# INDA25PlusPlus/rsoderh-raytracing

Hardware: AMD Instinct MI355X
Metric: Mrays/s, house.toml 1920x1080 256spp 8-bounce (higher is better)
Workload: dtype f32; 1 GPU; house.toml 1920x1080 256 spp 8 bounces, synthetic 2048x1024 HDRI env; parallelism=single GPU

## Files before the change

rsoderh-raytracing_amd/csrc/hip/rt_wavepool.h:

```cpp
#pragma once
#include "rt_device.h"
#include "rt_coop.h"
#include "rt_cold_layout.h"

enum HotField { H_OX, H_OY, H_OZ, H_EX, H_EY, H_EZ, H_SX, H_SY, H_SZ, H_T, H_CT, H_COUNT };
enum CtBits : uint32_t {
    F_SHADOW = 8u,
    F_EXT = 16u,
    F_NEE = 32u,
    F_OCCLUDED = 64u,
    CT_FLAGS = 120u,
    CT_SHIFT = 7u
};
#define RT_FLAT_BOUNCE_SHIFT 8u
#define RT_FLAT_BOUNCE_BITS 0xffff00u
#define RT_FLAT_RESUMED (1u << 24)
#define RT_FLAT_MAX_BOUNCES 0xffffu
static_assert(kColdWideStack == RT_WSTACK && kColdWideStateWords == RT_WSTATE_WORDS && kColdCoopOverflow == RT_COOP_GCAP,
              "rt_cold_layout.h sizes the walks' columns by the walks' own constants");
enum PoolTag { TAG_FREE = 0, TAG_TRACE = 1, TAG_MISS = 2, TAG_SHADE = 3, TAG_FINISH = 4, TAG_IDLE = 6 };
enum PoolStage { ST_GEN = 0, ST_TRACE = 1, ST_MISS = 2, ST_SHADE = 3, ST_FINISH = 4, ST_COUNT = 5 };

__host__ __device__ constexpr uint32_t pool_hot_columns(int trav) { return trav == 6 ? 12u : (uint32_t)H_COUNT; }
__host__ __device__ constexpr uint32_t pool_list_dwords(int trav) { return trav == 6 ? RT_COOP_LCAP : 64u; }
__host__ __device__ constexpr uint32_t pool_wave_lds_dwords(int trav, uint32_t pool) { return pool_hot_columns(trav) * pool + pool_list_dwords(trav) + (trav == 6 ? RT_COOP_NCAP + RT_COOP_MAP : 0u); }
template <uint32_t POOL, int TRAV>
struct PoolLayout {
    static constexpr uint32_t kSlotsPerLane = (POOL + 63u) / 64u;
    static constexpr uint32_t kHotDwords = pool_hot_columns(TRAV) * POOL;
    static constexpr uint32_t kListDwords = pool_list_dwords(TRAV);
    static constexpr uint32_t kWaveLdsDwords = pool_wave_lds_dwords(TRAV, POOL);
    static constexpr uint32_t kColdColumns = pool_cold_columns(TRAV);
    static constexpr uint32_t kWaveColdDwords = pool_wave_cold_dwords(TRAV, POOL);
    static constexpr uint32_t kCtColumn = pool_hot_columns(TRAV) - 1u;
};

RT_DEV uint32_t stage_of_tag(uint32_t tag) { return tag; }

#define RT_WAVE_HANDOVER()                                        \
    do {                                                          \
        __builtin_amdgcn_fence(__ATOMIC_RELEASE, "wavefront");    \
        __builtin_amdgcn_wave_barrier();                          \
        __builtin_amdgcn_fence(__ATOMIC_ACQUIRE, "wavefront");    \
    } while (0)

typedef float rt_f3v __attribute__((ext_vector_type(3)));
typedef rt_f3v rt_f3v_a4 __attribute__((aligned(4)));
RT_DEV void store_sample(float *dst, V3 L) { __builtin_nontemporal_store(rt_f3v{L.x, L.y, L.z}, reinterpret_cast<rt_f3v_a4 *>(dst)); }

#ifndef RT_POOL_WAVES_PER_SIMD
#define RT_POOL_WAVES_PER_SIMD 4
#endif
template <int SV> struct PoolView;
template <> struct PoolView<0> { typedef SceneView<false> type; static __device__ __forceinline__ type make(const DevScene &sc) { return make_view<false>(sc); } };
template <> struct PoolView<1> { typedef SceneView<true> type; static __device__ __forceinline__ type make(const DevScene &sc) { return make_view<true>(sc); } };
template <> struct PoolView<2> { typedef SceneViewHybrid type; static __device__ __forceinline__ type make(const DevScene &sc) { return make_view_hybrid(sc); } };

template <int SV, uint32_t BLOCK, uint32_t POOL, int TRAV>
__global__ __launch_bounds__(BLOCK, RT_POOL_WAVES_PER_SIMD) void rt_render_pool_kernel(RenderParams P)
{
    typedef PoolLayout<POOL, TRAV> L;
    constexpr bool kCoop = TRAV == 6;
    constexpr bool kBounceInCt = TRAV == 2;
    constexpr bool kFreshInCt = kBounceInCt;
    constexpr bool kOutHot = kFreshInCt;
    constexpr bool kRngHot = TRAV == 2;
    constexpr uint32_t kTCell = kRngHot ? (uint32_t)H_SX : (uint32_t)H_T;
    constexpr bool kFlatVote = kRngHot && kBounceInCt;
    constexpr bool kPackedMiss = TRAV == 2 || TRAV == 6;
    constexpr bool kGenTrace = TRAV >= 2 && !kCoop;
    const DevScene &sc = P.scene;
    if (SV != 0) stage_scene_lds(sc);
    const typename PoolView<SV>::type S = PoolView<SV>::make(sc);
    const uint32_t lane0 = threadIdx.x & (RT_WAVE - 1);
    constexpr bool kScalarWave = SV == 2 || TRAV == 6;
    const uint32_t wave = kScalarWave ? (uint32_t)__builtin_amdgcn_readfirstlane((int)(threadIdx.x / RT_WAVE)) : threadIdx.x / RT_WAVE;
    uint32_t *const lds32 = reinterpret_cast<uint32_t *>(rt_smem + sc.lds_float4s);
    uint32_t *const W = lds32 + wave * L::kWaveLdsDwords;
    uint32_t *const WCT = W + L::kCtColumn * POOL;
    uint32_t *const list = W + L::kHotDwords;
    uint32_t *const G = P.cold_state + (size_t)(blockIdx.x * (BLOCK / RT_WAVE) + wave) * L::kWaveColdDwords;
    const bool prune = (P.flags & RSRT_FLAG_PRUNE) != 0;
    const bool anyhit_shadow = !(P.flags & RSRT_FLAG_REFERENCE_TRAVERSAL);
    const uint32_t tile_px = P.tile_w * P.tile_h;

#define HOT(f, slot) W[(f) * POOL + (slot)]
#define HOTF(f, slot) as_f(HOT(f, slot))
#define SETHU(f, slot, val) W[(f) * POOL + (slot)] = (val)
#define SETH(f, slot, val) SETHU(f, slot, as_u(val))
#define CT_OF(slot) WCT[(slot)]
#define TAG_OF(slot) (WCT[(slot)] & 7u)
#define SET_TAG(slot, tag) WCT[(slot)] = (uint32_t)(tag)
#define SET_CT(slot, payload, flags, tag) WCT[(slot)] = ((payload) << CT_SHIFT) | (flags) | (uint32_t)(tag)
#define BEST_REF(slot) W[9u * POOL + 2u * (slot)]
#define BEST_T(slot) W[9u * POOL + 2u * (slot) + 1u]
#define COLD(f, slot) G[cold_index(TRAV, POOL, (f), (slot))]
#define COLDF(f, slot) as_f(COLD(f, slot))
#define SETC(f, slot, val) COLD(f, slot) = as_u(val)

    for (uint32_t k = 0; k < L::kSlotsPerLane; k++)
        if (lane0 + 64u * k < POOL) SET_TAG(lane0 + 64u * k, TAG_FREE);
    RT_WAVE_HANDOVER();

    uint32_t chunk_next = 0, chunk_left = 0, chunk_tile_slot0 = 0, chunk_tx0 = 0, chunk_ty0 = 0, chunk_s0 = 0, chunk_p0 = 0;
    bool exhausted = false;
    unsigned long long n_paths = 0, n_ext = 0, n_shadow = 0;
    uint32_t n_work = 0;
#ifdef RT_INSTRUMENT
    DbgCounters dbg;
    for (int i = 0; i < RT_DBG_N; i++) dbg.c[i] = 0;
#endif

#ifdef RT_INSTRUMENT
    unsigned long long t_prev = __builtin_amdgcn_s_memtime();
#define DBG_STAMP(i) do { unsigned long long t_now = __builtin_amdgcn_s_memtime(); if (lane0 == 0) dbg.c[i] += t_now - t_prev; t_prev = t_now; } while (0)
#else
#define DBG_STAMP(i) do { } while (0)
#endif
#if defined(RT_INSTRUMENT) && defined(RT_SHADE_PROFILE)
#define SHADE_STAMP(i) DBG_STAMP(i)
#else
#define SHADE_STAMP(i) do { } while (0)
#endif
    auto ray_end = [&](const uint32_t slot, const uint32_t ct, const Hit &h, const uint32_t cur, const float t_in, const unsigned long long flat_rem) __attribute__((always_inline)) {
        const bool shadow = (ct & F_SHADOW) != 0u;
        const uint32_t bounce_bits = kBounceInCt ? ((ct >> CT_SHIFT) & RT_FLAT_BOUNCE_BITS) : 0u;
        const bool found = TRAV >= 3 ? (h.ref != RT_REF_UNKNOWN) : (h.t < t_in);
        const bool done = cur == RT_END || (kFlatVote && shadow && h.t < RT_INFINITY);
        if (!done && kFlatVote) {
            COLD(C_REM_LO, slot) = (uint32_t)flat_rem;
            COLD(C_REM_HI, slot) = (uint32_t)(flat_rem >> 32);
            if (!shadow) SETH(kTCell, slot, h.t);
            SET_CT(slot, RT_FLAT_RESUMED | bounce_bits | (shadow ? 0u : h.ref), ct & CT_FLAGS, TAG_TRACE);
        } else if (!done) {
            if (!kRngHot) SETH(H_T, slot, h.t);
            if (TRAV != 2 && !shadow && found) COLD(C_REF, slot) = h.ref;
            SET_CT(slot, cur, ct & CT_FLAGS, TAG_TRACE);
        } else if (shadow) {
            n_shadow++;
            if (!kRngHot) SETH(H_T, slot, RT_INFINITY);
            const uint32_t fl = (ct & (F_EXT | F_NEE)) | (h.t < RT_INFINITY ? (uint32_t)F_OCCLUDED : 0u);
            SET_CT(slot, bounce_bits, fl, (ct & F_EXT) ? TAG_TRACE : TAG_FINISH);
        } else {
            n_ext++;
            SETH(kTCell, slot, h.t);
            if (TRAV != 2 && found) COLD(C_REF, slot) = h.ref;
            SET_CT(slot, (TRAV == 2 ? h.ref : 0u) | bounce_bits, ct & (F_NEE | F_OCCLUDED), h.did_hit() ? TAG_SHADE : TAG_MISS);
        }
    };
    auto trace_slot = [&](const uint32_t slot, const uint32_t ct, const V3 o, const V3 d, const bool coherent) __attribute__((always_inline)) {
        const bool shadow = (ct & F_SHADOW) != 0u;
        Hit h;
        uint32_t cur = kBounceInCt ? (kFlatVote ? (ct >> (CT_SHIFT + 24u)) : 0u) : (ct >> CT_SHIFT);
        h.src = SRC_BVH;
        h.t = kRngHot ? RT_INFINITY : HOTF(H_T, slot); h.u = h.v = 0.0f;
        unsigned long long flat_rem = 0ull;
        if (kFlatVote && cur != 0u) {
            flat_rem = ((unsigned long long)COLD(C_REM_HI, slot) << 32) | COLD(C_REM_LO, slot);
            if (!shadow) h.t = HOTF(kTCell, slot);
        }
        h.ref = (TRAV >= 3 && !shadow) ? RT_REF_UNKNOWN : ((kFlatVote && cur != 0u) ? ((ct >> CT_SHIFT) & 63u) : 0u);
        const float t_in = h.t;
        trace_dispatch<TRAV>(DBG_ARG S, sc, o, d, prune, shadow && anyhit_shadow, P.trace_budget, TRAV == 2 ? (kFlatVote ? P.flat_quorum : 0u) : P.descend_quorum,
                             cur, h, TRAV == 2 ? nullptr : &COLD(C_REF, slot), n_work, flat_rem, TRAV >= 4 ? &G[C_WIDE_STATE * POOL + slot] : nullptr, POOL, P.stop_quorum, coherent);
        ray_end(slot, ct, h, cur, t_in, flat_rem);
    };
    for (;;) {
        uint32_t lane = lane0;
        if (kCoop) asm volatile("" : "+v"(lane));
        RT_MARK(0);
        DBG_STAMP(21);
        uint32_t tags[L::kSlotsPerLane];
        uint32_t count[ST_COUNT] = {};
        for (uint32_t k = 0; k < L::kSlotsPerLane; k++) {
            tags[k] = (lane + 64u * k < POOL) ? TAG_OF(lane + 64u * k) : (uint32_t)TAG_IDLE;
            const uint32_t st = stage_of_tag(tags[k]);
            for (uint32_t s = 0; s < ST_COUNT; s++) count[s] += (uint32_t)__popcll(__ballot(st == s));
        }
        if (exhausted) count[ST_GEN] = 0;
        uint32_t best = ST_COUNT, best_n = 0;
        for (uint32_t s = 0; s < ST_COUNT; s++)
            if (count[s] >= best_n && count[s] > 0) { best = s; best_n = count[s]; }
        if (best == ST_COUNT) break;
        uint32_t base = 0;
        for (uint32_t k = 0; k < L::kSlotsPerLane; k++) {
            const bool mine = stage_of_tag(tags[k]) == best;
            const unsigned long long m = __ballot(mine);
            const uint32_t pos = base + (uint32_t)__popcll(m & ((1ull << lane) - 1ull));
            if (mine && pos < L::kListDwords) list[pos] = lane + 64u * k;
            base += (uint32_t)__popcll(m);
        }
        RT_WAVE_HANDOVER();
        const uint32_t n_run = min(best_n, 64u);
        const bool on = lane < n_run;
        const uint32_t slot = on ? list[lane] : 0u;
        const uint32_t dbg_stage = best;
        (void)dbg_stage;
        if (lane == 0) { DBG_ADD(dbg_stage, 1); DBG_ADD(5 + dbg_stage, (kCoop && best == ST_TRACE) ? best_n : n_run); }
        DBG_STAMP(22);
        RT_MARK(1);

        if (best == ST_GEN) {
            RT_MARK(2);
            uint32_t given = 0;
            bool started = false;
            V3 cam_o = v3(0.0f, 0.0f, 0.0f), cam_d = v3(0.0f, 0.0f, 0.0f);
            while (given < n_run && !exhausted) {
                if (chunk_left == 0u) {
                    uint32_t c = 0;
                    if (lane == 0) c = atomicAdd(P.work_counter, 1u);
                    c = __builtin_amdgcn_readfirstlane((int)c);
                    if (c >= P.n_chunks) { exhausted = true; break; }
                    const uint32_t q = c % P.n_subtiles, cb = c / P.n_subtiles;
                    const uint32_t j = cb / P.n_sblocks, b = cb % P.n_sblocks;
                    uint32_t ttx, tty;
                    if (!owned_tile(j, P.rank, P.world, P.skew, P.tiles_x, P.tiles_per_row, ttx, tty)) continue;
                    chunk_tx0 = ttx * P.tile_w;
                    chunk_ty0 = tty * P.tile_h;
                    chunk_tile_slot0 = j * tile_px;
                    chunk_s0 = b * P.samples_per_chunk;
                    chunk_p0 = q * P.chunk_px;
                    chunk_next = 0;
                    chunk_left = min(P.samples_per_chunk, P.sample_count - chunk_s0) * P.chunk_px;
                }
                const uint32_t take = min(n_run - given, chunk_left);
                if (on && lane >= given && lane < given + take) {
                    const uint32_t item = chunk_next + (lane - given);
                    const uint32_t ks = item / P.chunk_px, p = chunk_p0 + item % P.chunk_px;
                    const uint32_t px = chunk_tx0 + p % P.tile_w, py = chunk_ty0 + p / P.tile_w;
                    if (px < P.width && py < P.height) {
                        const uint32_t srel = chunk_s0 + ks;
                        PathState ps;
                        start_path(P, px, py, P.sample_begin + srel, ps);
                        SETH(H_OX, slot, ps.o.x); SETH(H_OY, slot, ps.o.y); SETH(H_OZ, slot, ps.o.z);
                        SETH(H_EX, slot, ps.d.x); SETH(H_EY, slot, ps.d.y); SETH(H_EZ, slot, ps.d.z);
                        if (kRngHot) SETHU(H_T, slot, ps.rng);
                        else if (!kCoop) SETH(H_T, slot, RT_INFINITY);
                        if (!kFreshInCt) {
                            SETC(C_TX, slot, 1.0f); SETC(C_TY, slot, 1.0f); SETC(C_TZ, slot, 1.0f);
                            SETC(C_LX, slot, 0.0f); SETC(C_LY, slot, 0.0f); SETC(C_LZ, slot, 0.0f);
                            SETC(C_LASTPDF, slot, 1.0f);
                        }
                        if (!kRngHot) COLD(C_RNG, slot) = ps.rng;
                        if (!kBounceInCt) COLD(C_BOUNCE, slot) = 0u;
                        if (kOutHot) SETHU(H_SY, slot, srel * P.n_slots + chunk_tile_slot0 + p);
                        else COLD(C_OUT, slot) = srel * P.n_slots + chunk_tile_slot0 + p;
                        if (kGenTrace) { started = true; cam_o = ps.o; cam_d = ps.d; }
                        else SET_CT(slot, 0u, F_EXT, TAG_TRACE);
                        n_paths++;
                    }
                }
                given += take;
                chunk_next += take;
                chunk_left -= take;
            }
            RT_MARK(3);
            if (kGenTrace && started) trace_slot(slot, (uint32_t)F_EXT | (uint32_t)TAG_TRACE, cam_o, cam_d, true);
            RT_MARK(14);
            if (exhausted) {
                for (uint32_t k = 0; k < L::kSlotsPerLane; k++)
                    if (lane + 64u * k < POOL && TAG_OF(lane + 64u * k) == TAG_FREE) SET_TAG(lane + 64u * k, TAG_IDLE);
            }
        } else if (kCoop && best == ST_TRACE) {
            if constexpr (kCoop) {
                CoopStacks cs;
                cs.ns = list + L::kListDwords; cs.ls = list; cs.gs = G + L::kColdColumns * POOL;
                cs.map = reinterpret_cast<uint16_t *>(cs.ns + RT_COOP_NCAP);
                cs.ns_h = cs.ns_n = cs.ls_n = cs.gs_n = 0u;
                cs.lds_cap = P.coop_lds_cap; cs.lifo_at = P.coop_lifo_at; cs.narrow_at = P.coop_narrow_at; cs.gcap = P.coop_gcap;
                CoopNoCount coop_cc;
                for (uint32_t i0 = 0; i0 < best_n; i0 += 64u) {
                    const bool valid = i0 + lane < best_n;
                    const uint32_t s = list[valid ? i0 + lane : 0u];
                    coop_push_rays<POOL>(W, cs, coop_cc, valid, s, CT_OF(s), (uint32_t)F_EXT, (uint32_t)F_SHADOW);
                }
                coop_trace<POOL>(DBG_ARG S, W, cs, coop_cc, anyhit_shadow, lane, n_work);
                RT_WAVE_HANDOVER();
                uint32_t my_slot[L::kSlotsPerLane];
                bool mine[L::kSlotsPerLane];
                for (uint32_t k = 0; k < L::kSlotsPerLane; k++) { my_slot[k] = lane + 64u * k; mine[k] = tags[k] == (uint32_t)TAG_TRACE; }
                if (cs.overflowed()) {
                    if (lane == 0u) atomicAdd(&P.stats[RT_COOP_STATS + 6u], 1ull);
                    for (uint32_t k = 0; k < L::kSlotsPerLane; k++)
                        if (mine[k]) coop_abandon<POOL>(W, my_slot[k], (uint32_t)F_EXT, (uint32_t)F_SHADOW);
                }
                coop_slow_rays<POOL, L::kSlotsPerLane>(DBG_ARG S, sc, W, mine, my_slot, anyhit_shadow, n_work);
                for (uint32_t k = 0; k < L::kSlotsPerLane; k++) {
                    if (!mine[k]) continue;
                    const uint32_t s = my_slot[k], ct = CT_OF(s);
                    const uint32_t fl = ct & (uint32_t)(F_NEE | F_OCCLUDED);
                    if (ct & F_SHADOW) n_shadow++;
                    if (ct & F_EXT) {
                        n_ext++;
                        SET_CT(s, 0u, fl, as_f(BEST_T(s)) < RT_INFINITY ? TAG_SHADE : TAG_MISS);
                    } else {
                        SET_CT(s, 0u, fl, TAG_FINISH);
                    }
                }
            }
        } else if (best == ST_TRACE) {
            RT_MARK(12);
            if (on) {
                const uint32_t ct = CT_OF(slot);
                const uint32_t dcol = (ct & F_SHADOW) ? (uint32_t)H_SX : (uint32_t)H_EX;
                const V3 o = v3(HOTF(H_OX, slot), HOTF(H_OY, slot), HOTF(H_OZ, slot));
                const V3 d = v3(HOTF(dcol, slot), HOTF(dcol + 1u, slot), HOTF(dcol + 2u, slot));
                trace_slot(slot, ct, o, d, false);
            }
        } else if (best == ST_MISS) {
            RT_MARK2(0);
            if (on) {
                const uint32_t ct = CT_OF(slot);
                const V3 o = v3(HOTF(H_OX, slot), HOTF(H_OY, slot), HOTF(H_OZ, slot));
                const V3 d = v3(HOTF(H_EX, slot), HOTF(H_EY, slot), HOTF(H_EZ, slot));
                float env_u, env_v;
                direction_to_equirectangular_uv(d, env_u, env_v);
                const EnvBilinearFetch sky_fetch = kPackedMiss ? sample_env_bilinear_begin_pmf(P.env, env_u, env_v) : sample_env_bilinear_begin(P.env, env_u, env_v);
                float sky_pmf = 0.0f;
                if (!kPackedMiss) sky_pmf = environment_direction_pmf(P.env, env_u, env_v);
                float last_pdf;
                V3 T, Lr, nee_prev;
                uint32_t out_slot;
                if constexpr (!kFreshInCt) {
                    last_pdf = COLDF(C_LASTPDF, slot);
                    T = v3(COLDF(C_TX, slot), COLDF(C_TY, slot), COLDF(C_TZ, slot));
                    Lr = v3(COLDF(C_LX, slot), COLDF(C_LY, slot), COLDF(C_LZ, slot));
                    nee_prev = v3(COLDF(C_NEEX, slot), COLDF(C_NEEY, slot), COLDF(C_NEEZ, slot));
                    out_slot = COLD(C_OUT, slot);
                } else {
                    const bool fresh = ((ct >> CT_SHIFT) & RT_FLAT_BOUNCE_BITS) == 0u;
                    const uint32_t out_hot = HOT(H_SY, slot);
                    last_pdf = COLDF(C_LASTPDF, slot);
                    T = v3(COLDF(C_TX, slot), COLDF(C_TY, slot), COLDF(C_TZ, slot));
                    Lr = v3(COLDF(C_LX, slot), COLDF(C_LY, slot), COLDF(C_LZ, slot));
                    nee_prev = v3(COLDF(C_NEEX, slot), COLDF(C_NEEY, slot), COLDF(C_NEEZ, slot));
                    out_slot = COLD(C_OUT, slot);
                    if (fresh) {
                        last_pdf = 1.0f;
                        T = v3(1.0f, 1.0f, 1.0f);
                        Lr = v3(0.0f, 0.0f, 0.0f);
                        out_slot = out_hot;
                    }
                }
                Hit h;
                h.t = RT_INFINITY; h.ref = 0; h.src = SRC_BVH; h.u = h.v = 0.0f;
                for (uint32_t i = 0; i < sc.n_spheres; i++) {
                    RT_MARK2(1);
                    float u, v;
                    float t = test_record(S, i, SRC_FB_SPHERE, o, d, u, v);
                    if (t >= 0.0f && t < h.t) { h.t = t; h.ref = i; h.src = SRC_FB_SPHERE; }
                }
                for (uint32_t i = 0; i < sc.n_planes; i++) {
                    RT_MARK2(2);
                    float u, v;
                    float t = test_record(S, i, SRC_FB_PLANE, o, d, u, v);
                    if (t >= 0.0f && t < h.t) { h.t = t; h.ref = i; h.src = SRC_FB_PLANE; }
                }
                RT_MARK2(3);
                if (h.did_hit()) {
                    if (kCoop) BEST_T(slot) = as_u(h.t); else SETH(kTCell, slot, h.t);
                    if (kCoop) {
                        BEST_REF(slot) = h.ref | (h.src << 30);
                        SET_CT(slot, 0u, ct & (F_NEE | F_OCCLUDED), TAG_SHADE);
                    } else if (TRAV == 2) {
                        SET_CT(slot, h.ref | (h.src << 6) | (kBounceInCt ? ((ct >> CT_SHIFT) & RT_FLAT_BOUNCE_BITS) : 0u), ct & (F_NEE | F_OCCLUDED), TAG_SHADE);
                    } else {
                        COLD(C_REF, slot) = h.ref | (h.src << 30);
                        SET_CT(slot, 0u, ct & (F_NEE | F_OCCLUDED), TAG_SHADE);
                    }
                } else {
                    const V3 sky = sample_env_bilinear_finish(sky_fetch);
                    if (kPackedMiss) sky_pmf = env_bilinear_pmf(P.env, sky_fetch, env_u, env_v);
                    const float pdf = sky_pmf / environment_pixel_solid_angle(env_v, P.env);
                    const float w = power_heuristic(last_pdf, pdf);
                    if ((ct & (F_NEE | F_OCCLUDED)) == F_NEE) Lr = Lr + nee_prev;
                    Lr = Lr + T * sky * w;
                    store_sample(P.sample_buf + (size_t)out_slot * 3u, Lr);
                    SET_TAG(slot, TAG_FREE);
                }
            }
        } else if (best == ST_SHADE) {
            RT_MARK2(4);
            if (on) {
                const uint32_t ct = CT_OF(slot);
                const V3 o = v3(HOTF(H_OX, slot), HOTF(H_OY, slot), HOTF(H_OZ, slot));
                const V3 d = v3(HOTF(H_EX, slot), HOTF(H_EY, slot), HOTF(H_EZ, slot));
                Hit h;
                h.t = kCoop ? as_f(BEST_T(slot)) : HOTF(kTCell, slot);
                if (TRAV == 2) {
                    const uint32_t hr = (ct >> CT_SHIFT) & 0xffu;
                    h.ref = hr & 63u; h.src = hr >> 6;
                } else {
                    const uint32_t hr = kCoop ? BEST_REF(slot) : COLD(C_REF, slot);
                    h.ref = hr & 0x3fffffffu; h.src = hr >> 30;
                }
                DBG_ADD(27, (as_u(hit_record(S, h, 0).w) & 3u) == PRIM_TRIANGLE ? 1 : 0); DBG_ADD(31, (as_u(hit_record(S, h, 0).w) & 3u) == PRIM_SPHERE ? 1 : 0);
                uint32_t rng, bounce;
                uint32_t out_slot = 0u;
                V3 T, Lr;
                Surface surf;
                BsdfMaterial mat;
                EnvironmentSample es;
                if constexpr (kRngHot) {
                    rng = HOT(H_T, slot);
                    const EnvironmentPick pick = sample_environment_begin(P.env, rng);
                    T = v3(COLDF(C_TX, slot), COLDF(C_TY, slot), COLDF(C_TZ, slot));
                    Lr = v3(COLDF(C_LX, slot), COLDF(C_LY, slot), COLDF(C_LZ, slot));
                    const V3 nee_prev = v3(COLDF(C_NEEX, slot), COLDF(C_NEEY, slot), COLDF(C_NEEZ, slot));
                    if (kOutHot) out_slot = COLD(C_OUT, slot);
                    bounce = (kBounceInCt ? (ct >> (CT_SHIFT + RT_FLAT_BOUNCE_SHIFT)) : COLD(C_BOUNCE, slot)) + 1u;
                    if (kFreshInCt && bounce == 1u) {
                        T = v3(1.0f, 1.0f, 1.0f);
                        Lr = v3(0.0f, 0.0f, 0.0f);
                        if (kOutHot) out_slot = HOT(H_SY, slot);
                    }
                    SHADE_STAMP(10);
                    hit_barycentrics(S, h, o, d);
                    surf = resolve_hit(S, h, o, d);
                    mat = load_material(S, surf.material_id);
                    SHADE_STAMP(11);
                    es = sample_environment_finish<true>(P.env, rng, pick);
                    SHADE_STAMP(12);
                    if ((ct & (F_NEE | F_OCCLUDED)) == F_NEE) Lr = Lr + nee_prev;
                    Lr = Lr + T * mat.emission;
                } else {
                    hit_barycentrics(S, h, o, d);
                    rng = COLD(C_RNG, slot);
                    T = v3(COLDF(C_TX, slot), COLDF(C_TY, slot), COLDF(C_TZ, slot));
                    Lr = v3(COLDF(C_LX, slot), COLDF(C_LY, slot), COLDF(C_LZ, slot));
                    bounce = (kBounceInCt ? (ct >> (CT_SHIFT + RT_FLAT_BOUNCE_SHIFT)) : COLD(C_BOUNCE, slot)) + 1u;
                    if ((ct & (F_NEE | F_OCCLUDED)) == F_NEE) Lr = Lr + v3(COLDF(C_NEEX, slot), COLDF(C_NEEY, slot), COLDF(C_NEEZ, slot));
                    surf = resolve_hit(S, h, o, d);
                    mat = load_material(S, surf.material_id);
                    Lr = Lr + T * mat.emission;
                    es = sample_environment(P.env, rng);
                }
                const float cos_nee = fmax_(0.0f, dot(surf.normal, es.direction));
                const bool want_shadow = cos_nee > 0.0f && es.pdf > 0.0f;
                const Frame frame = make_frame(surf.normal);
                const V3 wo = to_frame_local(frame, -d);
                V3 nee = v3(0.0f, 0.0f, 0.0f);
                const float g1_o = kRngHot ? g1_ggx(wo.z, mat.alpha) : 0.0f;
                if (want_shadow) {
                    RT_MARK2(5);
                    DBG_WAVE_TICK(23); DBG_ADD(24, 1);
                    const V3 wi = to_frame_local(frame, es.direction);
                    V3 scattering;
                    float pdf_bsdf;
                    if (kRngHot) bsdf_eval_pdf_local<true>(wo, wi, mat, g1_o, scattering, pdf_bsdf);
                    else bsdf_eval_pdf_local(wo, wi, mat, scattering, pdf_bsdf);
                    const float w = power_heuristic(es.pdf, pdf_bsdf);
                    nee = T * w * es.radiance * scattering * cos_nee / es.pdf;
                }
                RT_MARK2(6);
                SHADE_STAMP(13);
                const BsdfSample bs = kRngHot ? bsdf_sample_in_frame<true>(d, surf.normal, frame, wo, mat, g1_o, rng) : bsdf_sample_in_frame(d, surf.normal, frame, wo, mat, rng);
                RT_MARK2(15);
                SHADE_STAMP(14);
                bool finished = false, nee_counts = want_shadow;
                if (bs.dir.x == 0.0f && bs.dir.y == 0.0f && bs.dir.z == 0.0f) {
                    Lr = bs.scattering;
                    nee_counts = false;
                    finished = true;
                } else if (bs.pdf <= 0.0f) {
                    finished = true;
                } else {
                    const float c = fmax_(0.0f, dot(surf.normal, bs.dir));
                    T = T * (bs.scattering * (c / bs.pdf));
                    if (length(T) < 0.001f) finished = true;
                }
                if (bounce >= P.max_bounces) finished = true;
                if (finished && !want_shadow) {
                    store_sample(P.sample_buf + (size_t)(kOutHot ? out_slot : COLD(C_OUT, slot)) * 3u, Lr);
                    SET_TAG(slot, TAG_FREE);
                } else {
                    SETC(C_LX, slot, Lr.x); SETC(C_LY, slot, Lr.y); SETC(C_LZ, slot, Lr.z);
                    if (kOutHot) COLD(C_OUT, slot) = out_slot;
                    if (nee_counts) { SETC(C_NEEX, slot, nee.x); SETC(C_NEEY, slot, nee.y); SETC(C_NEEZ, slot, nee.z); }
                    if (!finished) {
                        SETC(C_LASTPDF, slot, bs.pdf);
                        SETC(C_TX, slot, T.x); SETC(C_TY, slot, T.y); SETC(C_TZ, slot, T.z);
                        if (kRngHot) SETHU(H_T, slot, rng); else COLD(C_RNG, slot) = rng;
                        if (!kBounceInCt) COLD(C_BOUNCE, slot) = bounce;
                        SETH(H_EX, slot, bs.dir.x); SETH(H_EY, slot, bs.dir.y); SETH(H_EZ, slot, bs.dir.z);
                    }
                    if (want_shadow) { SETH(H_SX, slot, es.direction.x); SETH(H_SY, slot, es.direction.y); SETH(H_SZ, slot, es.direction.z); }
                    SETH(H_OX, slot, surf.point.x); SETH(H_OY, slot, surf.point.y); SETH(H_OZ, slot, surf.point.z);
                    if (!kRngHot && !kCoop) SETH(H_T, slot, RT_INFINITY);
                    SET_CT(slot, kBounceInCt ? (bounce << RT_FLAT_BOUNCE_SHIFT) : 0u,
                           (want_shadow ? (uint32_t)F_SHADOW : 0u) | (finished ? 0u : (uint32_t)F_EXT) | (nee_counts ? (uint32_t)F_NEE : 0u), TAG_TRACE);
                }
            }
        } else {
            RT_MARK2(7);
            if (on) {
                const uint32_t ct = CT_OF(slot);
                V3 Lr = v3(COLDF(C_LX, slot), COLDF(C_LY, slot), COLDF(C_LZ, slot));
                if ((ct & (F_NEE | F_OCCLUDED)) == F_NEE) Lr = Lr + v3(COLDF(C_NEEX, slot), COLDF(C_NEEY, slot), COLDF(C_NEEZ, slot));
                store_sample(P.sample_buf + (size_t)COLD(C_OUT, slot) * 3u, Lr);
                SET_TAG(slot, TAG_FREE);
            }
        }
        RT_MARK(15);
        RT_WAVE_HANDOVER();
        DBG_STAMP(16 + dbg_stage);
    }
#undef HOT
#undef HOTF
#undef SETHU
#undef SETH
#undef CT_OF
#undef TAG_OF
#undef SET_TAG
#undef SET_CT
#undef COLD
#undef BEST_REF
#undef BEST_T
#undef COLDF
#undef SETC

    RT_MARK(11);
    unsigned long long n_work64 = n_work;
    for (int off = 32; off > 0; off >>= 1) {
        n_paths += __shfl_down(n_paths, off);
        n_ext += __shfl_down(n_ext, off);
        n_shadow += __shfl_down(n_shadow, off);
        if (TRAV != 2) n_work64 += __shfl_down(n_work64, off);
    }
    if (lane0 == 0) {
        atomicAdd(&P.stats[0], n_paths);
        atomicAdd(&P.stats[1], n_ext);
        atomicAdd(&P.stats[2], n_shadow);
        if (TRAV != 2) atomicAdd(&P.stats[3], n_work64);
    }
#ifdef RT_INSTRUMENT
    for (int i = 0; i < RT_DBG_N; i++) {
        unsigned long long v = dbg.c[i];
        for (int off = 32; off > 0; off >>= 1) v += __shfl_down(v, off);
        if (lane0 == 0 && v) atomicAdd(&P.stats[4 + i], v);
    }
#endif
}
```

Measured before the change: 23240 Mrays/s.

## Track per-stage slot counts incrementally and pick stage via packed max key

For the TRAV==2 wavefront pool, the scheduler now keeps running per-stage counts and updates them after each stage from ballots over only the slots that just ran, instead of re-ballotting every pool slot against every stage each iteration. Stage selection becomes a packed (count<<3|stage) max chain kept in scalar registers, and list compaction uses mbcnt instead of a masked popcount. This is meant to cut scheduler overhead per iteration, at the cost of bookkeeping that must stay exactly in step with tag transitions. Only the default TRAV==2 path uses it, if that is the active traversal.

```diff
diff --git a/rsoderh-raytracing_amd/csrc/hip/rt_pool_pick.h b/rsoderh-raytracing_amd/csrc/hip/rt_pool_pick.h
--- /dev/null
+++ b/rsoderh-raytracing_amd/csrc/hip/rt_pool_pick.h
@@ -0,0 +1,39 @@
+#pragma once
+#include <cstdint>
+
+#if defined(__HIPCC__) || defined(__CUDACC__)
+#define RT_PICK_FN __host__ __device__ inline
+#else
+#define RT_PICK_FN inline
+#endif
+#if defined(__HIP_DEVICE_COMPILE__)
+#define RT_PICK_SCALAR(x) asm volatile("" : "+s"(x))
+#else
+#define RT_PICK_SCALAR(x) (void)(x)
+#endif
+
+constexpr uint32_t kPoolPickStages = 5u;
+
+struct PoolPick {
+    uint32_t best;
+    uint32_t best_n;
+};
+
+RT_PICK_FN uint32_t pool_pick_max(uint32_t a, uint32_t b) { return a > b ? a : b; }
+
+RT_PICK_FN PoolPick pool_pick(uint32_t n_gen, uint32_t n_trace, uint32_t n_miss, uint32_t n_shade, uint32_t n_finish, bool exhausted)
+{
+    uint32_t key = exhausted ? 0u : (n_gen << 3);
+    key = pool_pick_max(key, (n_trace << 3) | 1u);
+    RT_PICK_SCALAR(key);
+    key = pool_pick_max(key, (n_miss << 3) | 2u);
+    RT_PICK_SCALAR(key);
+    key = pool_pick_max(key, (n_shade << 3) | 3u);
+    RT_PICK_SCALAR(key);
+    key = pool_pick_max(key, (n_finish << 3) | 4u);
+    RT_PICK_SCALAR(key);
+    PoolPick p;
+    p.best = key < 8u ? kPoolPickStages : (key & 7u);
+    p.best_n = key >> 3;
+    return p;
+}
diff --git a/rsoderh-raytracing_amd/csrc/hip/rt_wavepool.h b/rsoderh-raytracing_amd/csrc/hip/rt_wavepool.h
--- a/rsoderh-raytracing_amd/csrc/hip/rt_wavepool.h
+++ b/rsoderh-raytracing_amd/csrc/hip/rt_wavepool.h
@@ -2,6 +2,7 @@
 #include "rt_device.h"
 #include "rt_coop.h"
 #include "rt_cold_layout.h"
+#include "rt_pool_pick.h"
 
 enum HotField { H_OX, H_OY, H_OZ, H_EX, H_EY, H_EZ, H_SX, H_SY, H_SZ, H_T, H_CT, H_COUNT };
 enum CtBits : uint32_t {
@@ -20,6 +21,7 @@
               "rt_cold_layout.h sizes the walks' columns by the walks' own constants");
 enum PoolTag { TAG_FREE = 0, TAG_TRACE = 1, TAG_MISS = 2, TAG_SHADE = 3, TAG_FINISH = 4, TAG_IDLE = 6 };
 enum PoolStage { ST_GEN = 0, ST_TRACE = 1, ST_MISS = 2, ST_SHADE = 3, ST_FINISH = 4, ST_COUNT = 5 };
+static_assert(ST_COUNT == kPoolPickStages, "rt_pool_pick.h picks among these stages, in this order");
 
 __host__ __device__ constexpr uint32_t pool_hot_columns(int trav) { return trav == 6 ? 12u : (uint32_t)H_COUNT; }
 __host__ __device__ constexpr uint32_t pool_list_dwords(int trav) { return trav == 6 ? RT_COOP_LCAP : 64u; }
@@ -69,6 +71,9 @@
     constexpr bool kFlatVote = kRngHot && kBounceInCt;
     constexpr bool kPackedMiss = TRAV == 2 || TRAV == 6;
     constexpr bool kGenTrace = TRAV >= 2 && !kCoop;
+    constexpr bool kKeptCounts = TRAV == 2;
+    constexpr bool kKeyPick = TRAV == 2;
+    constexpr bool kMbcnt = TRAV == 2;
     const DevScene &sc = P.scene;
     if (SV != 0) stage_scene_lds(sc);
     const typename PoolView<SV>::type S = PoolView<SV>::make(sc);
@@ -104,6 +109,8 @@
 
     uint32_t chunk_next = 0, chunk_left = 0, chunk_tile_slot0 = 0, chunk_tx0 = 0, chunk_ty0 = 0, chunk_s0 = 0, chunk_p0 = 0;
     bool exhausted = false;
+    uint32_t kept[ST_COUNT] = {POOL, 0u, 0u, 0u, 0u};
+    (void)kept;
     unsigned long long n_paths = 0, n_ext = 0, n_shadow = 0;
     uint32_t n_work = 0;
 #ifdef RT_INSTRUMENT
@@ -172,22 +179,42 @@
         DBG_STAMP(21);
         uint32_t tags[L::kSlotsPerLane];
         uint32_t count[ST_COUNT] = {};
-        for (uint32_t k = 0; k < L::kSlotsPerLane; k++) {
-            tags[k] = (lane + 64u * k < POOL) ? TAG_OF(lane + 64u * k) : (uint32_t)TAG_IDLE;
-            const uint32_t st = stage_of_tag(tags[k]);
-            for (uint32_t s = 0; s < ST_COUNT; s++) count[s] += (uint32_t)__popcll(__ballot(st == s));
+        if constexpr (kKeptCounts) {
+            for (uint32_t k = 0; k < L::kSlotsPerLane; k++)
+                tags[k] = (lane + 64u * k < POOL) ? TAG_OF(lane + 64u * k) : (uint32_t)TAG_IDLE;
+            for (uint32_t s = 0; s < ST_COUNT; s++) count[s] = kept[s];
+#ifdef RT_INSTRUMENT
+            for (uint32_t s = 0; s < ST_COUNT; s++) {
+                uint32_t n = 0;
+                for (uint32_t k = 0; k < L::kSlotsPerLane; k++) n += (uint32_t)__popcll(__ballot(stage_of_tag(tags[k]) == s));
+                if (lane == 0 && !(exhausted && s == ST_GEN) && n != count[s]) DBG_ADD(26, 1);
+            }
+#endif
+        } else {
+            for (uint32_t k = 0; k < L::kSlotsPerLane; k++) {
+                tags[k] = (lane + 64u * k < POOL) ? TAG_OF(lane + 64u * k) : (uint32_t)TAG_IDLE;
+                const uint32_t st = stage_of_tag(tags[k]);
+                for (uint32_t s = 0; s < ST_COUNT; s++) count[s] += (uint32_t)__popcll(__ballot(st == s));
+            }
         }
-        if (exhausted) count[ST_GEN] = 0;
         uint32_t best = ST_COUNT, best_n = 0;
-        for (uint32_t s = 0; s < ST_COUNT; s++)
-            if (count[s] >= best_n && count[s] > 0) { best = s; best_n = count[s]; }
-        if (best == ST_COUNT) break;
+        if constexpr (kKeyPick) {
+            const PoolPick pick = pool_pick(count[ST_GEN], count[ST_TRACE], count[ST_MISS], count[ST_SHADE], count[ST_FINISH], exhausted);
+            best = pick.best; best_n = pick.best_n;
+        } else {
+            if (exhausted) count[ST_GEN] = 0;
+            for (uint32_t s = 0; s < ST_COUNT; s++)
+                if (count[s] >= best_n && count[s] > 0) { best = s; best_n = count[s]; }
+        }
+        if (kKeyPick ? best_n == 0u : best == ST_COUNT) break;
         uint32_t base = 0;
         for (uint32_t k = 0; k < L::kSlotsPerLane; k++) {
             const bool mine = stage_of_tag(tags[k]) == best;
             const unsigned long long m = __ballot(mine);
-            const uint32_t pos = base + (uint32_t)__popcll(m & ((1ull << lane) - 1ull));
-            if (mine && pos < L::kListDwords) list[pos] = lane + 64u * k;
+            const uint32_t below = kMbcnt ? __builtin_amdgcn_mbcnt_hi((uint32_t)(m >> 32), __builtin_amdgcn_mbcnt_lo((uint32_t)m, 0u))
+                                          : (uint32_t)__popcll(m & ((1ull << lane) - 1ull));
+            const uint32_t pos = base + below;
+            if (mine && ((kMbcnt && k == 0u && L::kListDwords >= 64u) || pos < L::kListDwords)) list[pos] = lane + 64u * k;
             base += (uint32_t)__popcll(m);
         }
         RT_WAVE_HANDOVER();
@@ -199,6 +226,22 @@
         if (lane == 0) { DBG_ADD(dbg_stage, 1); DBG_ADD(5 + dbg_stage, (kCoop && best == ST_TRACE) ? best_n : n_run); }
         DBG_STAMP(22);
         RT_MARK(1);
+        auto settle = [&](const uint32_t from, const uint32_t exits, const bool rest) __attribute__((always_inline)) {
+            if constexpr (kKeptCounts) {
+                RT_WAVE_HANDOVER();
+                const uint32_t now = on ? TAG_OF(slot) : (uint32_t)TAG_IDLE;
+                kept[from] -= n_run;
+                uint32_t left = n_run;
+                for (uint32_t s = 0; s < ST_COUNT; s++) {
+                    if (!((exits >> s) & 1u)) continue;
+                    if (rest && (exits >> (s + 1u)) == 0u) { kept[s] += left; break; }
+                    const uint32_t n = (uint32_t)__popcll(__ballot(stage_of_tag(now) == s));
+                    kept[s] += n;
+                    left -= n;
+                }
+            }
+        };
+#define EXIT(st) (1u << (st))
 
         if (best == ST_GEN) {
             RT_MARK(2);
@@ -261,6 +304,8 @@
                 for (uint32_t k = 0; k < L::kSlotsPerLane; k++)
                     if (lane + 64u * k < POOL && TAG_OF(lane + 64u * k) == TAG_FREE) SET_TAG(lane + 64u * k, TAG_IDLE);
             }
+            settle(ST_GEN, EXIT(ST_GEN) | EXIT(ST_TRACE) | EXIT(ST_MISS) | EXIT(ST_SHADE), false);
+            if (exhausted) kept[ST_GEN] = 0u;
         } else if (kCoop && best == ST_TRACE) {
             if constexpr (kCoop) {
                 CoopStacks cs;
@@ -307,6 +352,7 @@
                 const V3 d = v3(HOTF(dcol, slot), HOTF(dcol + 1u, slot), HOTF(dcol + 2u, slot));
                 trace_slot(slot, ct, o, d, false);
             }
+            settle(ST_TRACE, EXIT(ST_TRACE) | EXIT(ST_MISS) | EXIT(ST_SHADE) | EXIT(ST_FINISH), true);
         } else if (best == ST_MISS) {
             RT_MARK2(0);
             if (on) {
@@ -379,6 +425,7 @@
                     SET_TAG(slot, TAG_FREE);
                 }
             }
+            settle(ST_MISS, EXIT(ST_GEN) | EXIT(ST_SHADE), true);
         } else if (best == ST_SHADE) {
             RT_MARK2(4);
             if (on) {
@@ -491,6 +538,7 @@
                            (want_shadow ? (uint32_t)F_SHADOW : 0u) | (finished ? 0u : (uint32_t)F_EXT) | (nee_counts ? (uint32_t)F_NEE : 0u), TAG_TRACE);
                 }
             }
+            settle(ST_SHADE, EXIT(ST_GEN) | EXIT(ST_TRACE), true);
         } else {
             RT_MARK2(7);
             if (on) {
@@ -500,11 +548,13 @@
                 store_sample(P.sample_buf + (size_t)COLD(C_OUT, slot) * 3u, Lr);
                 SET_TAG(slot, TAG_FREE);
             }
+            settle(ST_FINISH, EXIT(ST_GEN), true);
         }
         RT_MARK(15);
         RT_WAVE_HANDOVER();
         DBG_STAMP(16 + dbg_stage);
     }
+#undef EXIT
 #undef HOT
 #undef HOTF
 #undef SETHU
```

Measured after the change: 23640 Mrays/s (median of 6 runs). 1.02x the previous value.
